# advimman/lama

Hardware: NVIDIA H100
Metric: images/sec FFCResNetGenerator @512x512 bs32 (higher is better)
Workload: dtype bf16x3(f32 accumulate)

## Files before the change

lama_b200/csrc/conv_tc.cu:

```cuda
#include <cuda.h>
#include <stdlib.h>

#include <type_traits>

#include "common.cuh"

namespace ffcb {
namespace {

constexpr int BM = 128;
constexpr int BK = 64;
constexpr int WG_K = 16;
constexpr int kThreads = 384;
constexpr int kConsumers = 256;
constexpr int kTileABytes = BM * BK * 2;
constexpr int kMaxStages = 8;
constexpr int kBarBytes = 1024;
constexpr int kSmemLimit = 227 * 1024;

struct TcParams {
  View out, addend;
  const float* shift;
  int N, act, addend_post;
  int BN, num_n_tiles;
  long long num_m_tiles;
  int stages;
  int flat;
  int TW, TH, tiles_x, tiles_y;
  int stride;
  int coord_off[2];
  int nseg;
  int a_il[2];
  const unsigned short* a_ptr[2];
  long long a_sg[2], a_lo[2];
  int a_tiles_per_image[2];
  int out_planar;
  int ring;
  int hints;
  int rr_dy0, rr_a_bytes, rr_w_bytes;
  int halo_a_bytes;
  signed char seg_taps[FFCB_MAX_KSEG];
  ffcb_kseg seg[FFCB_MAX_KSEG];
};

__device__ __forceinline__ uint32_t smem_u32(const void* p) { return (uint32_t)__cvta_generic_to_shared(p); }

__device__ __forceinline__ void mbar_init(uint64_t* bar, uint32_t count) {
  asm volatile("mbarrier.init.shared::cta.b64 [%0], %1;" ::"r"(smem_u32(bar)), "r"(count));
}
__device__ __forceinline__ void mbar_expect_tx(uint64_t* bar, uint32_t bytes) {
  asm volatile("mbarrier.arrive.expect_tx.shared::cta.b64 _, [%0], %1;" ::"r"(smem_u32(bar)), "r"(bytes) : "memory");
}
__device__ __forceinline__ void mbar_arrive(uint64_t* bar) {
  asm volatile("mbarrier.arrive.shared::cta.b64 _, [%0];" ::"r"(smem_u32(bar)) : "memory");
}
__device__ __forceinline__ void mbar_wait(uint64_t* bar, uint32_t parity) {
  asm volatile(
      "{\n\t"
      ".reg .pred p;\n\t"
      "WAIT_LOOP:\n\t"
      "mbarrier.try_wait.parity.shared::cta.b64 p, [%0], %1;\n\t"
      "@p bra WAIT_DONE;\n\t"
      "bra WAIT_LOOP;\n\t"
      "WAIT_DONE:\n\t"
      "}\n" ::"r"(smem_u32(bar)), "r"(parity)
      : "memory");
}

__device__ __forceinline__ void tma_load_3d(void* dst, const CUtensorMap* map, uint64_t* bar, int c0, int c1, int c2) {
  asm volatile(
      "cp.async.bulk.tensor.3d.shared::cluster.global.mbarrier::complete_tx::bytes [%0], [%1, {%3, %4, %5}], [%2];"
      ::"r"(smem_u32(dst)), "l"(map), "r"(smem_u32(bar)), "r"(c0), "r"(c1), "r"(c2)
      : "memory");
}
__device__ __forceinline__ void tma_load_5d(void* dst, const CUtensorMap* map, uint64_t* bar, int c0, int c1, int c2,
                                            int c3, int c4) {
  asm volatile(
      "cp.async.bulk.tensor.5d.shared::cluster.global.mbarrier::complete_tx::bytes [%0], [%1, {%3, %4, %5, %6, %7}], [%2];"
      ::"r"(smem_u32(dst)), "l"(map), "r"(smem_u32(bar)), "r"(c0), "r"(c1), "r"(c2), "r"(c3), "r"(c4)
      : "memory");
}

__device__ __forceinline__ void bulk_load(void* dst, const void* src, uint32_t bytes, uint64_t* bar) {
  asm volatile("cp.async.bulk.shared::cluster.global.mbarrier::complete_tx::bytes [%0], [%1], %2, [%3];"
               ::"r"(smem_u32(dst)), "l"(src), "r"(bytes), "r"(smem_u32(bar)) : "memory");
}

__device__ __forceinline__ void prefetch_tmap(const CUtensorMap* map) {
  asm volatile("prefetch.tensormap [%0];" ::"l"(map) : "memory");
}

constexpr uint32_t kLoSw = 1u << 16;
constexpr uint32_t kHiSw = (uint32_t)(1024 >> 4) | (1u << 30);
constexpr uint32_t kLoIl = (uint32_t)(2048 >> 4) << 16;
constexpr uint32_t kHiIl = (uint32_t)(128 >> 4);

__device__ __forceinline__ uint32_t desc_addr(uint32_t saddr) { return (saddr & 0x3FFFF) >> 4; }

__device__ __forceinline__ uint64_t desc64(uint32_t lo, uint32_t hi) {
  uint64_t d;
  asm("mov.b64 %0, {%1, %2};" : "=l"(d) : "r"(lo), "r"(hi));
  return d;
}
__device__ __forceinline__ bool elect_one() {
  uint32_t pred;
  asm volatile(
      "{\n\t"
      ".reg .pred P;\n\t"
      "elect.sync _|P, 0xffffffff;\n\t"
      "selp.b32 %0, 1, 0, P;\n\t"
      "}\n"
      : "=r"(pred));
  return pred != 0;
}

__device__ __forceinline__ void wgmma_fence() { asm volatile("wgmma.fence.sync.aligned;" ::: "memory"); }
__device__ __forceinline__ void wgmma_commit() { asm volatile("wgmma.commit_group.sync.aligned;" ::: "memory"); }
template <int N>
__device__ __forceinline__ void wgmma_wait() { asm volatile("wgmma.wait_group.sync.aligned %0;" ::"n"(N) : "memory"); }
template <int BN>
__device__ __forceinline__ void fence_acc(float* d) {
#pragma unroll
  for (int i = 0; i < BN / 2; ++i) asm volatile("" : "+f"(d[i])::"memory");
}

__device__ __forceinline__ void wgmma_n32(float* d, uint64_t da, uint64_t db, uint32_t scale_d) {
  asm volatile(
      "{\n\t.reg .pred p;\n\tsetp.ne.b32 p, %18, 0;\n\t"
      "wgmma.mma_async.sync.aligned.m64n32k16.f32.bf16.bf16 {"
      "%0, %1, %2, %3, %4, %5, %6, %7, %8, %9, %10, %11, %12, %13, %14, %15"
      "}, %16, %17, p, 1, 1, 0, 0;\n\t}\n"
      : "+f"(d[0]), "+f"(d[1]), "+f"(d[2]), "+f"(d[3]), "+f"(d[4]), "+f"(d[5]), "+f"(d[6]), "+f"(d[7]),
        "+f"(d[8]), "+f"(d[9]), "+f"(d[10]), "+f"(d[11]), "+f"(d[12]), "+f"(d[13]), "+f"(d[14]), "+f"(d[15])
      : "l"(da), "l"(db), "r"(scale_d));
}
__device__ __forceinline__ void wgmma_n64(float* d, uint64_t da, uint64_t db, uint32_t scale_d) {
  asm volatile(
      "{\n\t.reg .pred p;\n\tsetp.ne.b32 p, %34, 0;\n\t"
      "wgmma.mma_async.sync.aligned.m64n64k16.f32.bf16.bf16 {"
      "%0, %1, %2, %3, %4, %5, %6, %7, %8, %9, %10, %11, %12, %13, %14, %15, "
      "%16, %17, %18, %19, %20, %21, %22, %23, %24, %25, %26, %27, %28, %29, %30, %31"
      "}, %32, %33, p, 1, 1, 0, 0;\n\t}\n"
      : "+f"(d[0]), "+f"(d[1]), "+f"(d[2]), "+f"(d[3]), "+f"(d[4]), "+f"(d[5]), "+f"(d[6]), "+f"(d[7]),
        "+f"(d[8]), "+f"(d[9]), "+f"(d[10]), "+f"(d[11]), "+f"(d[12]), "+f"(d[13]), "+f"(d[14]), "+f"(d[15]),
        "+f"(d[16]), "+f"(d[17]), "+f"(d[18]), "+f"(d[19]), "+f"(d[20]), "+f"(d[21]), "+f"(d[22]), "+f"(d[23]),
        "+f"(d[24]), "+f"(d[25]), "+f"(d[26]), "+f"(d[27]), "+f"(d[28]), "+f"(d[29]), "+f"(d[30]), "+f"(d[31])
      : "l"(da), "l"(db), "r"(scale_d));
}
__device__ __forceinline__ void wgmma_n96(float* d, uint64_t da, uint64_t db, uint32_t scale_d) {
  asm volatile(
      "{\n\t.reg .pred p;\n\tsetp.ne.b32 p, %50, 0;\n\t"
      "wgmma.mma_async.sync.aligned.m64n96k16.f32.bf16.bf16 {"
      "%0, %1, %2, %3, %4, %5, %6, %7, %8, %9, %10, %11, %12, %13, %14, %15, "
      "%16, %17, %18, %19, %20, %21, %22, %23, %24, %25, %26, %27, %28, %29, %30, %31, "
      "%32, %33, %34, %35, %36, %37, %38, %39, %40, %41, %42, %43, %44, %45, %46, %47"
      "}, %48, %49, p, 1, 1, 0, 0;\n\t}\n"
      : "+f"(d[0]), "+f"(d[1]), "+f"(d[2]), "+f"(d[3]), "+f"(d[4]), "+f"(d[5]), "+f"(d[6]), "+f"(d[7]),
        "+f"(d[8]), "+f"(d[9]), "+f"(d[10]), "+f"(d[11]), "+f"(d[12]), "+f"(d[13]), "+f"(d[14]), "+f"(d[15]),
        "+f"(d[16]), "+f"(d[17]), "+f"(d[18]), "+f"(d[19]), "+f"(d[20]), "+f"(d[21]), "+f"(d[22]), "+f"(d[23]),
        "+f"(d[24]), "+f"(d[25]), "+f"(d[26]), "+f"(d[27]), "+f"(d[28]), "+f"(d[29]), "+f"(d[30]), "+f"(d[31]),
        "+f"(d[32]), "+f"(d[33]), "+f"(d[34]), "+f"(d[35]), "+f"(d[36]), "+f"(d[37]), "+f"(d[38]), "+f"(d[39]),
        "+f"(d[40]), "+f"(d[41]), "+f"(d[42]), "+f"(d[43]), "+f"(d[44]), "+f"(d[45]), "+f"(d[46]), "+f"(d[47])
      : "l"(da), "l"(db), "r"(scale_d));
}
__device__ __forceinline__ void wgmma_n128(float* d, uint64_t da, uint64_t db, uint32_t scale_d) {
  asm volatile(
      "{\n\t.reg .pred p;\n\tsetp.ne.b32 p, %66, 0;\n\t"
      "wgmma.mma_async.sync.aligned.m64n128k16.f32.bf16.bf16 {"
      "%0, %1, %2, %3, %4, %5, %6, %7, %8, %9, %10, %11, %12, %13, %14, %15, "
      "%16, %17, %18, %19, %20, %21, %22, %23, %24, %25, %26, %27, %28, %29, %30, %31, "
      "%32, %33, %34, %35, %36, %37, %38, %39, %40, %41, %42, %43, %44, %45, %46, %47, "
      "%48, %49, %50, %51, %52, %53, %54, %55, %56, %57, %58, %59, %60, %61, %62, %63"
      "}, %64, %65, p, 1, 1, 0, 0;\n\t}\n"
      : "+f"(d[0]), "+f"(d[1]), "+f"(d[2]), "+f"(d[3]), "+f"(d[4]), "+f"(d[5]), "+f"(d[6]), "+f"(d[7]),
        "+f"(d[8]), "+f"(d[9]), "+f"(d[10]), "+f"(d[11]), "+f"(d[12]), "+f"(d[13]), "+f"(d[14]), "+f"(d[15]),
        "+f"(d[16]), "+f"(d[17]), "+f"(d[18]), "+f"(d[19]), "+f"(d[20]), "+f"(d[21]), "+f"(d[22]), "+f"(d[23]),
        "+f"(d[24]), "+f"(d[25]), "+f"(d[26]), "+f"(d[27]), "+f"(d[28]), "+f"(d[29]), "+f"(d[30]), "+f"(d[31]),
        "+f"(d[32]), "+f"(d[33]), "+f"(d[34]), "+f"(d[35]), "+f"(d[36]), "+f"(d[37]), "+f"(d[38]), "+f"(d[39]),
        "+f"(d[40]), "+f"(d[41]), "+f"(d[42]), "+f"(d[43]), "+f"(d[44]), "+f"(d[45]), "+f"(d[46]), "+f"(d[47]),
        "+f"(d[48]), "+f"(d[49]), "+f"(d[50]), "+f"(d[51]), "+f"(d[52]), "+f"(d[53]), "+f"(d[54]), "+f"(d[55]),
        "+f"(d[56]), "+f"(d[57]), "+f"(d[58]), "+f"(d[59]), "+f"(d[60]), "+f"(d[61]), "+f"(d[62]), "+f"(d[63])
      : "l"(da), "l"(db), "r"(scale_d));
}
template <int BN>
__device__ __forceinline__ void wgmma_bn(float* d, uint64_t da, uint64_t db, uint32_t scale_d) {
  static_assert(BN == 32 || BN == 64 || BN == 96 || BN == 128, "N tile");
  if constexpr (BN == 32) wgmma_n32(d, da, db, scale_d);
  else if constexpr (BN == 64) wgmma_n64(d, da, db, scale_d);
  else if constexpr (BN == 96) wgmma_n96(d, da, db, scale_d);
  else wgmma_n128(d, da, db, scale_d);
}

struct TileCoord {
  int b, y0, x0;
  long long m0;
};

__device__ __forceinline__ TileCoord tile_coord(const TcParams& p, long long m_tile) {
  TileCoord t;
  if (p.flat) {
    t.m0 = m_tile * BM;
    t.b = 0; t.y0 = 0; t.x0 = 0;
  } else {
    const int per_img = p.tiles_x * p.tiles_y;
    t.b = (int)(m_tile / per_img);
    const int r = (int)(m_tile - (long long)t.b * per_img);
    t.y0 = (r / p.tiles_x) * p.TH;
    t.x0 = (r % p.tiles_x) * p.TW;
    t.m0 = 0;
  }
  return t;
}

template <bool IL, bool PO, bool RR, bool HALO, int BN>
__global__ void __launch_bounds__(kThreads, 1)
conv_tc_kernel(const __grid_constant__ TcParams p, const __grid_constant__ CUtensorMap map_in0,
               const __grid_constant__ CUtensorMap map_in1, const __grid_constant__ CUtensorMap map_w) {
  extern __shared__ __align__(1024) uint8_t smem_raw[];
  uint8_t* smem = reinterpret_cast<uint8_t*>((reinterpret_cast<uintptr_t>(smem_raw) + 1023) & ~(uintptr_t)1023);
  const int w_bytes = p.BN * BK * 2;
  const int stage_bytes = RR ? 2 * p.rr_a_bytes : HALO ? 2 * w_bytes : 2 * kTileABytes + 2 * w_bytes;
  uint8_t* w_res = smem;
  uint8_t* a_buf = smem;
  if constexpr (RR) smem += p.rr_w_bytes;
  if constexpr (HALO) smem += (size_t)4 * p.halo_a_bytes;
  uint64_t* bars = reinterpret_cast<uint64_t*>(smem + (size_t)p.stages * stage_bytes);
  uint64_t* full = bars;
  uint64_t* empty = bars + kMaxStages;
  uint64_t* w_bar = bars + 2 * kMaxStages;
  uint64_t* a_full = bars + 2 * kMaxStages + 1;
  uint64_t* a_empty = a_full + 2;

  const int warp = threadIdx.x >> 5, lane = threadIdx.x & 31;

  if (warp == 0 && lane == 0) {
    prefetch_tmap(&map_in0);
    prefetch_tmap(&map_in1);
    prefetch_tmap(&map_w);
  }
  if (warp == 1 && lane == 0) {
    for (int s = 0; s < p.stages; ++s) { mbar_init(&full[s], 1); mbar_init(&empty[s], kConsumers); }
    if constexpr (RR) mbar_init(w_bar, 1);
    if constexpr (HALO)
      for (int s = 0; s < 2; ++s) { mbar_init(&a_full[s], 1); mbar_init(&a_empty[s], kConsumers); }
    asm volatile("fence.mbarrier_init.release.cluster;" ::: "memory");
  }
  __syncthreads();

  int total_kblocks = 0;
  for (int s = 0; s < p.nseg; ++s) total_kblocks += (p.seg[s].nch + BK - 1) / BK;
  const long long num_tiles = p.num_m_tiles * p.num_n_tiles;

  if (warp == 0) {
    if constexpr (HALO) {
      int stage = 0, ast = 0;
      uint32_t phase = 0, aph = 0;
      for (long long t = blockIdx.x; t < num_tiles; t += gridDim.x) {
        const int n_tile = (int)(t % p.num_n_tiles);
        const TileCoord tc = tile_coord(p, t / p.num_n_tiles);
        int kofs = 0;
        for (int s = 0; s < p.nseg;) {
          const int ntap = p.seg_taps[s];
          const ffcb_kseg g = p.seg[s];
          const CUtensorMap* map = g.src ? &map_in1 : &map_in0;
          const int nblk = (g.nch + BK - 1) / BK;
          for (int j = 0; j < nblk; ++j) {
            for (int u = 0; u < (ntap == 9 ? 3 : 1); ++u) {
              const int dxu = ntap == 9 ? u - 1 : g.dx;
              mbar_wait(&a_empty[ast], aph ^ 1);
              if (elect_one()) {
                uint8_t* ab = a_buf + (size_t)ast * 2 * p.halo_a_bytes;
                mbar_expect_tx(&a_full[ast], 2u * p.TW * (p.TH + 2) * BK * 2);
                const int cx = tc.x0 + dxu + p.coord_off[g.src], cy = tc.y0 - 1 + p.coord_off[g.src];
                tma_load_5d(ab, map, &a_full[ast], g.c0 + j * BK, cx, cy, tc.b, 0);
                tma_load_5d(ab + p.halo_a_bytes, map, &a_full[ast], g.c0 + j * BK, cx, cy, tc.b, 1);
              }
              __syncwarp();
              if (++ast == 2) { ast = 0; aph ^= 1; }
              for (int tap = 0; tap < ntap; ++tap) {
                if (p.seg[s + tap].dx != dxu) continue;
                mbar_wait(&empty[stage], phase ^ 1);
                if (elect_one()) {
                  uint8_t* st = smem + (size_t)stage * stage_bytes;
                  mbar_expect_tx(&full[stage], (uint32_t)stage_bytes);
                  const int k = kofs + (tap * nblk + j) * BK;
                  tma_load_3d(st, &map_w, &full[stage], k, n_tile * p.BN, 0);
                  tma_load_3d(st + w_bytes, &map_w, &full[stage], k, n_tile * p.BN, 1);
                }
                __syncwarp();
                if (++stage == p.stages) { stage = 0; phase ^= 1; }
              }
            }
          }
          kofs += ntap * nblk * BK;
          s += ntap;
        }
      }
    } else if constexpr (RR) {
      const ffcb_kseg g0 = p.seg[0];
      const CUtensorMap* map = g0.src ? &map_in1 : &map_in0;
      if (elect_one()) {
        mbar_expect_tx(w_bar, (uint32_t)p.rr_w_bytes);
        for (int s = 0; s < p.nseg; ++s) {
          tma_load_3d(w_res + (size_t)s * 2 * w_bytes, &map_w, w_bar, s * BK, 0, 0);
          tma_load_3d(w_res + (size_t)s * 2 * w_bytes + w_bytes, &map_w, w_bar, s * BK, 0, 1);
        }
      }
      __syncwarp();
      int stage = 0;
      uint32_t phase = 0;
      for (long long t = blockIdx.x; t < num_tiles; t += gridDim.x) {
        const TileCoord tc = tile_coord(p, t);
        mbar_wait(&empty[stage], phase ^ 1);
        if (elect_one()) {
          uint8_t* st = smem + (size_t)stage * stage_bytes;
          mbar_expect_tx(&full[stage], (uint32_t)stage_bytes);
          const int cx = tc.x0 + g0.dx + p.coord_off[g0.src], cy = tc.y0 + p.rr_dy0 + p.coord_off[g0.src];
          tma_load_5d(st, map, &full[stage], g0.c0, cx, cy, tc.b, 0);
          tma_load_5d(st + p.rr_a_bytes, map, &full[stage], g0.c0, cx, cy, tc.b, 1);
        }
        __syncwarp();
        if (++stage == p.stages) { stage = 0; phase ^= 1; }
      }
    } else {
      int stage = 0;
      uint32_t phase = 0;
      for (long long t = blockIdx.x; t < num_tiles; t += gridDim.x) {
        const int n_tile = (int)(t % p.num_n_tiles);
        const TileCoord tc = tile_coord(p, t / p.num_n_tiles);
        int kb = 0;
        for (int s = 0; s < p.nseg; ++s) {
          const ffcb_kseg g = p.seg[s];
          const CUtensorMap* map = g.src ? &map_in1 : &map_in0;
          const int nblk = (g.nch + BK - 1) / BK;
          const int cx = tc.x0 * p.stride + g.dx + p.coord_off[g.src];
          const int cy = tc.y0 * p.stride + g.dy + p.coord_off[g.src];
          const int il = IL ? p.a_il[g.src] : 0;
          for (int j = 0; j < nblk; ++j, ++kb) {
            mbar_wait(&empty[stage], phase ^ 1);
            if (elect_one()) {
              uint8_t* st = smem + (size_t)stage * stage_bytes;
              mbar_expect_tx(&full[stage], (uint32_t)stage_bytes);
              const int cc = g.c0 + j * BK;
              if (IL && il) {
                const long long blk = p.flat ? (tc.m0 >> 7)
                                             : (long long)tc.b * p.a_tiles_per_image[g.src] + ((tc.y0 * p.out.W) >> 7);
                const unsigned short* src = p.a_ptr[g.src] + blk * p.a_sg[g.src] + (long long)(cc >> 3) * 1024;
                bulk_load(st, src, kTileABytes, &full[stage]);
                bulk_load(st + kTileABytes, src + p.a_lo[g.src], kTileABytes, &full[stage]);
              } else if (p.flat) {
                tma_load_3d(st, map, &full[stage], cc, (int)tc.m0, 0);
                tma_load_3d(st + kTileABytes, map, &full[stage], cc, (int)tc.m0, 1);
              } else {
                tma_load_5d(st, map, &full[stage], cc, cx, cy, tc.b, 0);
                tma_load_5d(st + kTileABytes, map, &full[stage], cc, cx, cy, tc.b, 1);
              }
              tma_load_3d(st + 2 * kTileABytes, &map_w, &full[stage], kb * BK, n_tile * p.BN, 0);
              tma_load_3d(st + 2 * kTileABytes + w_bytes, &map_w, &full[stage], kb * BK, n_tile * p.BN, 1);
            }
            __syncwarp();
            if (++stage == p.stages) { stage = 0; phase ^= 1; }
          }
        }
      }
    }
  } else if (warp >= 4) {
    const int g = (warp >> 2) - 1;
    const int w = warp & 3, q = lane & 3;
    const int row = g * 64 + w * 16 + (lane >> 2) + 8 * (q & 1);
    const int cb = 4 * (q >> 1);
    const bool odd = (q & 1) != 0;
    const uint32_t a_row_sw = (uint32_t)(g * 64 * BK * 2) >> 4;
    const uint32_t a_row_il = (uint32_t)(g * 64 * 16) >> 4;
    const int HW = p.out.H * p.out.W;
    const bool has_add = p.addend.ptr != nullptr;
    float acc[BN / 2];
#pragma unroll
    for (int i = 0; i < BN / 2; ++i) acc[i] = 0.f;
    int stage = 0, ast = 0;
    uint32_t phase = 0, aph = 0;
    const int a_row0 = (g + 1) * p.TW;
    if constexpr (RR) mbar_wait(w_bar, 0);
    for (long long t = blockIdx.x; t < num_tiles; t += gridDim.x) {
      const int n_tile = (int)(t % p.num_n_tiles);
      const TileCoord tc = tile_coord(p, t / p.num_n_tiles);
      fence_acc<BN>(acc);
      if constexpr (HALO) {
        int prev = -1, a_prev = -1, nt = 0;
        for (int s = 0; s < p.nseg;) {
          const int ntap = p.seg_taps[s];
          const int nblk = (p.seg[s].nch + BK - 1) / BK;
          for (int j = 0; j < nblk; ++j) {
            for (int u = 0; u < (ntap == 9 ? 3 : 1); ++u) {
              const int dxu = ntap == 9 ? u - 1 : p.seg[s].dx;
              mbar_wait(&a_full[ast], aph);
              const uint32_t ab = smem_u32(a_buf + (size_t)ast * 2 * p.halo_a_bytes);
              for (int tap = 0; tap < ntap; ++tap) {
                const int dy = p.seg[s + tap].dy;
                if (p.seg[s + tap].dx != dxu) continue;
                const uint32_t a_off = (uint32_t)((a_row0 + dy * p.TW) * (BK * 2)) >> 4;
                const uint32_t a_hi = desc_addr(ab) + a_off;
                const uint32_t a_lo = desc_addr(ab + (uint32_t)p.halo_a_bytes) + a_off;
                mbar_wait(&full[stage], phase);
                wgmma_fence();
                const uint32_t st = smem_u32(smem + (size_t)stage * stage_bytes);
                const uint32_t w_hi = desc_addr(st), w_lo = desc_addr(st + (uint32_t)w_bytes);
#pragma unroll
                for (int k = 0; k < BK / WG_K; ++k) {
                  const uint32_t adv = (uint32_t)((k * WG_K * 2) >> 4);
                  wgmma_bn<BN>(acc, desc64((a_hi + adv) | kLoSw, kHiSw), desc64((w_hi + adv) | kLoSw, kHiSw),
                               (nt | k) != 0);
                  wgmma_bn<BN>(acc, desc64((a_lo + adv) | kLoSw, kHiSw), desc64((w_hi + adv) | kLoSw, kHiSw), 1);
                  wgmma_bn<BN>(acc, desc64((a_hi + adv) | kLoSw, kHiSw), desc64((w_lo + adv) | kLoSw, kHiSw), 1);
                }
                wgmma_commit();
                wgmma_wait<1>();
                if (prev >= 0) mbar_arrive(&empty[prev]);
                prev = stage;
                if (++stage == p.stages) { stage = 0; phase ^= 1; }
                if (a_prev >= 0) { mbar_arrive(&a_empty[a_prev]); a_prev = -1; }
                ++nt;
              }
              a_prev = ast;
              if (++ast == 2) { ast = 0; aph ^= 1; }
            }
          }
          s += ntap;
        }
        wgmma_wait<0>();
        fence_acc<BN>(acc);
        mbar_arrive(&empty[prev]);
        mbar_arrive(&a_empty[a_prev]);
      } else if constexpr (RR) {
        mbar_wait(&full[stage], phase);
        const uint32_t st = smem_u32(smem + (size_t)stage * stage_bytes);
        const uint32_t wr = smem_u32(w_res);
        for (int sgi = 0; sgi < p.nseg; ++sgi) {
          wgmma_fence();
          const uint32_t a_off = (uint32_t)((p.seg[sgi].dy - p.rr_dy0) * p.TW * (BK * 2));
          const uint32_t a_hi = desc_addr(st + a_off) + a_row_sw;
          const uint32_t a_lo = desc_addr(st + a_off + (uint32_t)p.rr_a_bytes) + a_row_sw;
          const uint32_t w_hi = desc_addr(wr + (uint32_t)(sgi * 2 * w_bytes));
          const uint32_t w_lo = desc_addr(wr + (uint32_t)(sgi * 2 * w_bytes + w_bytes));
#pragma unroll
          for (int k = 0; k < BK / WG_K; ++k) {
            const uint32_t adv = (uint32_t)((k * WG_K * 2) >> 4);
            wgmma_bn<BN>(acc, desc64((a_hi + adv) | kLoSw, kHiSw), desc64((w_hi + adv) | kLoSw, kHiSw), (sgi | k) != 0);
            wgmma_bn<BN>(acc, desc64((a_lo + adv) | kLoSw, kHiSw), desc64((w_hi + adv) | kLoSw, kHiSw), 1);
            wgmma_bn<BN>(acc, desc64((a_hi + adv) | kLoSw, kHiSw), desc64((w_lo + adv) | kLoSw, kHiSw), 1);
          }
          wgmma_commit();
          wgmma_wait<1>();
        }
        wgmma_wait<0>();
        fence_acc<BN>(acc);
        mbar_arrive(&empty[stage]);
        if (++stage == p.stages) { stage = 0; phase ^= 1; }
      } else {
        int prev = -1, sgi = 0, j = 0;
        for (int kb = 0; kb < total_kblocks; ++kb) {
          const bool il = IL && p.a_il[p.seg[sgi].src] != 0;
          const uint32_t a_lodesc = il ? kLoIl : kLoSw, a_hidesc = il ? kHiIl : kHiSw;
          const uint32_t a_row = il ? a_row_il : a_row_sw;
          const uint32_t a_step = il ? (uint32_t)(4096 >> 4) : (uint32_t)((WG_K * 2) >> 4);
          if (IL && ++j == (p.seg[sgi].nch + BK - 1) / BK) { ++sgi; j = 0; }
          mbar_wait(&full[stage], phase);
          wgmma_fence();
          const uint32_t st = smem_u32(smem + (size_t)stage * stage_bytes);
          const uint32_t a_hi = desc_addr(st) + a_row;
          const uint32_t a_lo = desc_addr(st + kTileABytes) + a_row;
          const uint32_t w_hi = desc_addr(st + 2 * kTileABytes);
          const uint32_t w_lo = desc_addr(st + 2 * kTileABytes + w_bytes);
#pragma unroll
          for (int k = 0; k < BK / WG_K; ++k) {
            const uint32_t wadv = (uint32_t)((k * WG_K * 2) >> 4);
            const uint32_t aadv = (uint32_t)k * a_step;
            wgmma_bn<BN>(acc, desc64((a_hi + aadv) | a_lodesc, a_hidesc), desc64((w_hi + wadv) | kLoSw, kHiSw),
                         (kb | k) != 0);
            wgmma_bn<BN>(acc, desc64((a_lo + aadv) | a_lodesc, a_hidesc), desc64((w_hi + wadv) | kLoSw, kHiSw), 1);
            wgmma_bn<BN>(acc, desc64((a_hi + aadv) | a_lodesc, a_hidesc), desc64((w_lo + wadv) | kLoSw, kHiSw), 1);
          }
          wgmma_commit();
          wgmma_wait<1>();
          if (prev >= 0) mbar_arrive(&empty[prev]);
          prev = stage;
          if (++stage == p.stages) { stage = 0; phase ^= 1; }
        }
        wgmma_wait<0>();
        fence_acc<BN>(acc);
        mbar_arrive(&empty[prev]);
      }

      int b, y, x;
      bool valid;
      if (p.flat) {
        const unsigned m = (unsigned)tc.m0 + (unsigned)row;
        valid = m < (unsigned)(p.out.B * HW);
        const unsigned mm = valid ? m : 0u;
        b = (int)(mm / (unsigned)HW);
        const unsigned r = mm - (unsigned)b * (unsigned)HW;
        y = (int)(r / (unsigned)p.out.W);
        x = (int)(r - (unsigned)y * (unsigned)p.out.W);
      } else {
        b = tc.b;
        y = tc.y0 + row / p.TW;
        x = tc.x0 + row % p.TW;
        valid = y < p.out.H && x < p.out.W;
      }
      const long long o_out = valid ? pix_off(p.out, b, y, x) : 0;
      const long long o_add = (has_add && valid) ? pix_off(p.addend, b, y, x) : 0;
      int mir_dy = 0, mir_dx = 0;
      if (!PO && p.ring && valid) {
        int my, mx;
        if (ring_mirrors(p.out, y, x, my, mx)) {
          if (my != -2) mir_dy = (my - y) * (int)p.out.sy;
          if (mx != -2) mir_dx = (mx - x) * (int)p.out.sx;
        }
      }
      const uint64_t pol = l2_policy(PO && p.hints ? 2 : 0);
#pragma unroll
      for (int j = 0; j < BN / 8; ++j) {
        const float s0 = odd ? acc[4 * j] : acc[4 * j + 2], s1 = odd ? acc[4 * j + 1] : acc[4 * j + 3];
        const float r0 = __shfl_xor_sync(0xffffffffu, s0, 1), r1 = __shfl_xor_sync(0xffffffffu, s1, 1);
        float4 v = odd ? make_float4(r0, r1, acc[4 * j + 2], acc[4 * j + 3])
                       : make_float4(acc[4 * j], acc[4 * j + 1], r0, r1);
        const int n = n_tile * p.BN + 8 * j + cb;
        if (!valid || n >= p.N) continue;
        if (p.shift != nullptr) {
          const float4 sh = __ldg(reinterpret_cast<const float4*>(p.shift + n));
          v.x += sh.x; v.y += sh.y; v.z += sh.z; v.w += sh.w;
        }
        float4 ad = make_float4(0.f, 0.f, 0.f, 0.f);
        if (has_add) ad = load4(p.addend, o_add + n);
        if (!p.addend_post) { v.x += ad.x; v.y += ad.y; v.z += ad.z; v.w += ad.w; }
        if (p.act == FFCB_ACT_RELU) {
          v.x = fmaxf(v.x, 0.f); v.y = fmaxf(v.y, 0.f); v.z = fmaxf(v.z, 0.f); v.w = fmaxf(v.w, 0.f);
        } else if (p.act != FFCB_ACT_NONE) {
          v.x = slow_act(v.x, p.act); v.y = slow_act(v.y, p.act); v.z = slow_act(v.z, p.act); v.w = slow_act(v.w, p.act);
        }
        if (p.addend_post) { v.x += ad.x; v.y += ad.y; v.z += ad.z; v.w += ad.w; }
        if constexpr (PO) {
          st_hint_f4(reinterpret_cast<float*>(p.out.ptr) + o_out + chan_off(p.out, n), v, pol);
        } else {
          store4(p.out, o_out + n, v);
          if (mir_dy) store4(p.out, o_out + mir_dy + n, v);
          if (mir_dx) store4(p.out, o_out + mir_dx + n, v);
          if (mir_dy && mir_dx) store4(p.out, o_out + mir_dy + mir_dx + n, v);
        }
      }
    }
  }
}

typedef CUresult (*EncodeTiledFn)(CUtensorMap*, CUtensorMapDataType, cuuint32_t, void*, const cuuint64_t*,
                                  const cuuint64_t*, const cuuint32_t*, const cuuint32_t*, CUtensorMapInterleave,
                                  CUtensorMapSwizzle, CUtensorMapL2promotion, CUtensorMapFloatOOBfill);

EncodeTiledFn get_encode() {
  static EncodeTiledFn fn = nullptr;
  if (fn == nullptr) {
    void* p = nullptr;
    cudaDriverEntryPointQueryResult q;
    if (cudaGetDriverEntryPoint("cuTensorMapEncodeTiled", &p, cudaEnableDefault, &q) == cudaSuccess &&
        q == cudaDriverEntryPointSuccess)
      fn = reinterpret_cast<EncodeTiledFn>(p);
  }
  return fn;
}

int encode_typed(CUtensorMap* map, void* base, CUtensorMapDataType dt, CUtensorMapSwizzle sw, int rank,
                 const cuuint64_t* dims, const cuuint64_t* strides_bytes, const cuuint32_t* box, const cuuint32_t* estr,
                 const char* what) {
  EncodeTiledFn fn = get_encode();
  if (fn == nullptr) {
    set_error("conv(tc): cuTensorMapEncodeTiled entry point unavailable");
    return FFCB_ECUDA;
  }
  CUresult r = fn(map, dt, (cuuint32_t)rank, base, dims, strides_bytes, box, estr, CU_TENSOR_MAP_INTERLEAVE_NONE, sw,
                  CU_TENSOR_MAP_L2_PROMOTION_L2_256B, CU_TENSOR_MAP_FLOAT_OOB_FILL_NONE);
  if (r != CUDA_SUCCESS) {
    set_error("conv(tc): cuTensorMapEncodeTiled(%s) failed with CUresult %d (rank %d, dims %llu %llu %llu, box %u %u %u)",
              what, (int)r, rank, (unsigned long long)dims[0], (unsigned long long)dims[1],
              (unsigned long long)(rank > 2 ? dims[2] : 0), box[0], box[1], rank > 2 ? box[2] : 0);
    return FFCB_ECUDA;
  }
  return FFCB_OK;
}

int encode(CUtensorMap* map, void* base, int rank, const cuuint64_t* dims, const cuuint64_t* strides_bytes,
           const cuuint32_t* box, const cuuint32_t* estr, const char* what) {
  return encode_typed(map, base, CU_TENSOR_MAP_DATA_TYPE_BFLOAT16, CU_TENSOR_MAP_SWIZZLE_128B, rank, dims, strides_bytes,
                      box, estr, what);
}

int pick_bn(int n) {
  if (const char* e = getenv("FFCB_TC_BN")) {
    const int v = atoi(e);
    if (v >= 32 && v <= 128 && v % 32 == 0) return v < n ? v : (n + 31) / 32 * 32;
  }
  if (n <= 128) return (n + 31) / 32 * 32;
  if (n == 192) return 96;
  return 128;
}

}

int conv_tc(const ffcb_conv_desc* d, cudaStream_t stream) {
  FFCB_REQUIRE(d->out.B > 0, "conv(tc): empty batch");
  FFCB_REQUIRE((long long)d->out.B * d->out.H * d->out.W < (1ll << 31), "conv(tc): more than 2^31 output pixels");
  bool used[2] = {false, false}, taps[2] = {false, false};
  int reach[2] = {0, 0};
  for (int i = 0; i < d->nseg; ++i) {
    used[d->seg[i].src] = true;
    if (d->seg[i].dx != 0 || d->seg[i].dy != 0) taps[d->seg[i].src] = true;
    const int ax = d->seg[i].dx < 0 ? -d->seg[i].dx : d->seg[i].dx, ay = d->seg[i].dy < 0 ? -d->seg[i].dy : d->seg[i].dy;
    if (ax > reach[d->seg[i].src]) reach[d->seg[i].src] = ax;
    if (ay > reach[d->seg[i].src]) reach[d->seg[i].src] = ay;
    FFCB_REQUIRE(d->seg[i].c0 % 8 == 0, "conv(tc): segment %d starts at channel %d (must be a multiple of 8)", i,
                 d->seg[i].c0);
  }
  for (int s = 0; s < 2; ++s) {
    if (!used[s]) continue;
    const ffcb_tensor& t = d->in[s];
    FFCB_REQUIRE(t.fmt == FFCB_BF16X2, "conv(tc): in[%d] must be split bf16 (FFCB_BF16X2)", s);
    if (t.cg != 0) {
      FFCB_REQUIRE(t.cg == 8 && t.tile == 128 && !taps[s] && d->stride == 1 && t.H == d->out.H && t.W == d->out.W,
                   "conv(tc): a channel-group planar in[%d] must be tile-blocked (tile=128, cg=8) with 1x1 taps, stride 1",
                   s);
      for (int i = 0; i < d->nseg; ++i)
        if (d->seg[i].src == s)
// ... 112 lines not shown
    p.num_m_tiles = (long long)d->out.B * p.tiles_x * p.tiles_y;
    p.halo_a_bytes = p.TW * (p.TH + 2) * BK * 2;
  } else {
    int tw = 1;
    while (tw < W && tw < BM) tw <<= 1;
    p.TW = tw; p.TH = BM / tw;
    p.tiles_x = (W + p.TW - 1) / p.TW;
    p.tiles_y = (H + p.TH - 1) / p.TH;
    p.num_m_tiles = (long long)d->out.B * p.tiles_x * p.tiles_y;
    FFCB_REQUIRE(p.TW * d->stride <= 256 && p.TH * d->stride <= 256, "conv(tc): tile exceeds the TMA box limit");
  }

  for (int s = 0; s < 2; ++s)
    if (p.a_il[s] && !flat)
      FFCB_REQUIRE(p.TW == W && p.TW * p.TH == BM && H % p.TH == 0 && (H * W) % BM == 0,
                   "conv(tc): tile-blocked in[%d] in a spatial contraction needs M tiles of whole rows (W a power of two "
                   "<= 128 dividing 128, H*W a multiple of 128); got %dx%d", s, H, W);

  alignas(64) CUtensorMap maps[3];
  int rc;
  for (int s = 0; s < 2; ++s) {
    if (!used[s]) { p.coord_off[s] = 0; continue; }
    const ffcb_tensor& t = d->in[s];
    const cuuint64_t esz = 2;
    if (p.a_il[s]) { p.coord_off[s] = 0; continue; }
    if (flat) {
      cuuint64_t dims[3] = {(cuuint64_t)t.C, (cuuint64_t)t.B * t.H * t.W, 2};
      cuuint64_t str[2] = {(cuuint64_t)t.sx * esz, (cuuint64_t)t.lo_off * esz};
      cuuint32_t box[3] = {BK, BM, 1}, es[3] = {1, 1, 1};
      p.coord_off[s] = 0;
      if ((rc = encode(&maps[s], t.ptr, 3, dims, str, box, es, "flat activations"))) return rc;
    } else {
      const bool ring = taps[s] && d->border == FFCB_BORDER_REFLECT;
      const int off = ring ? t.pad : 0;
      char* base = (char*)t.ptr - (int64_t)off * ((int64_t)t.sy + t.sx) * (int64_t)esz;
      cuuint64_t dims[5] = {(cuuint64_t)t.C, (cuuint64_t)(t.W + 2 * off), (cuuint64_t)(t.H + 2 * off),
                            (cuuint64_t)t.B, 2};
      cuuint64_t str[4] = {(cuuint64_t)t.sx * esz, (cuuint64_t)t.sy * esz, (cuuint64_t)t.sb * esz,
                           (cuuint64_t)t.lo_off * esz};
      cuuint32_t box[5] = {BK, (cuuint32_t)(p.TW * d->stride), (cuuint32_t)(p.TH * d->stride), 1, 1};
      if (rr) box[2] = (cuuint32_t)(p.TH + rr_dy_max - rr_dy_min);
      if (halo) box[2] = (cuuint32_t)(p.TH + 2);
      cuuint32_t es[5] = {1, (cuuint32_t)d->stride, (cuuint32_t)d->stride, 1, 1};
      p.coord_off[s] = off;
      if ((rc = encode(&maps[s], base, 5, dims, str, box, es, "spatial activations"))) return rc;
    }
  }
  {
    cuuint64_t dims[3] = {(cuuint64_t)kpad, (cuuint64_t)d->n_out, 2};
    cuuint64_t str[2] = {(cuuint64_t)kpad * 2, (cuuint64_t)kpad * d->n_out * 2};
    cuuint32_t box[3] = {BK, (cuuint32_t)p.BN, 1}, es[3] = {1, 1, 1};
    FFCB_REQUIRE(((uintptr_t)d->weight % 16) == 0, "conv(tc): weight pointer not 16-byte aligned");
    if ((rc = encode(&maps[2], const_cast<void*>(d->weight), 3, dims, str, box, es, "weights"))) return rc;
  }

  for (int s = 0; s < 2; ++s)
    if (!used[s] || p.a_il[s]) maps[s] = maps[2];
  if (d->out.cg == 0) {
    const ffcb_tensor& t = d->out;
    const cuuint64_t esz = t.fmt == FFCB_BF16X2 ? 2 : 4;
    FFCB_REQUIRE(((uintptr_t)t.ptr % 16) == 0 && (t.sx * esz) % 16 == 0 && (t.sy * esz) % 16 == 0 &&
                     (t.sb * esz) % 16 == 0 && (esz == 4 || (t.lo_off * esz) % 16 == 0),
                 "conv(tc): out strides / pointer not 16-byte aligned (C must be a multiple of %d)", esz == 2 ? 8 : 4);
  }

  const int stage_bytes = rr ? 2 * p.rr_a_bytes : halo ? 2 * p.BN * BK * 2 : 2 * kTileABytes + 2 * p.BN * BK * 2;
  const int bar_bytes = kBarBytes + (rr ? p.rr_w_bytes : 0) + (halo ? 4 * p.halo_a_bytes : 0);
  int stages = (kSmemLimit - 1024 - bar_bytes) / stage_bytes;
  if (stages > kMaxStages) stages = kMaxStages;
  FFCB_REQUIRE(stages >= 2, "conv(tc): BN=%d leaves fewer than 2 pipeline stages", p.BN);
  p.stages = stages;
  const size_t smem = (size_t)stages * stage_bytes + bar_bytes + 1024;
  int dev = 0, sms = 132;
  FFCB_CUDA(cudaGetDevice(&dev));
  FFCB_CUDA(cudaDeviceGetAttribute(&sms, cudaDevAttrMultiProcessorCount, dev));
  const long long tiles = p.num_m_tiles * p.num_n_tiles;
  const int grid = (int)(tiles < sms ? tiles : sms);
  const bool any_il = p.a_il[0] || p.a_il[1];
  auto launch = [&](auto kernel) -> int {
    FFCB_CUDA(cudaFuncSetAttribute(kernel, cudaFuncAttributeMaxDynamicSharedMemorySize, kSmemLimit));
    kernel<<<grid, kThreads, smem, stream>>>(p, maps[0], maps[1], maps[2]);
    return FFCB_OK;
  };
  auto launch_bn = [&](auto bn) -> int {
    constexpr int N = decltype(bn)::value;
    if (rr) return launch(conv_tc_kernel<false, false, true, false, N>);
    if (halo) return launch(conv_tc_kernel<false, false, false, true, N>);
    if (any_il)
      return p.out_planar ? launch(conv_tc_kernel<true, true, false, false, N>)
                          : launch(conv_tc_kernel<true, false, false, false, N>);
    return p.out_planar ? launch(conv_tc_kernel<false, true, false, false, N>)
                        : launch(conv_tc_kernel<false, false, false, false, N>);
  };
  switch (p.BN) {
    case 32: rc = launch_bn(std::integral_constant<int, 32>()); break;
    case 64: rc = launch_bn(std::integral_constant<int, 64>()); break;
    case 96: rc = launch_bn(std::integral_constant<int, 96>()); break;
    default: rc = launch_bn(std::integral_constant<int, 128>()); break;
  }
  if (rc) return rc;
  FFCB_LAUNCH_CHECK("conv_tc_kernel");
  return FFCB_OK;
}

}
```

Baseline: 314.7.

## Add ping-pong consumer warpgroup schedule with register reallocation to tensor-core conv

For flat and row-reuse conv modes, the two consumer warpgroups now each own whole 128-row tiles and alternate tiles, rather than splitting one tile's rows. Named barriers order their MMA phases so one warpgroup's epilogue overlaps the other's mainloop. Producer warps drop registers via setmaxnreg and consumers raise theirs to hold two accumulator sets. The goal is to hide epilogue cost behind tensor-core work, at the price of doubled accumulator registers and more complex ring/phase bookkeeping.

Result: no change. 316.0, median of 6 (+0.4%).

```diff
diff --git a/lama_b200/csrc/conv_tc.cu b/lama_b200/csrc/conv_tc.cu
--- a/lama_b200/csrc/conv_tc.cu
+++ b/lama_b200/csrc/conv_tc.cu
@@ -4,6 +4,7 @@
 #include <type_traits>
 
 #include "common.cuh"
+#include "conv_tc_sched.cuh"
 
 namespace ffcb {
 namespace {
@@ -12,7 +13,9 @@
 constexpr int BK = 64;
 constexpr int WG_K = 16;
 constexpr int kThreads = 384;
-constexpr int kConsumers = 256;
+constexpr int kProducerRegs = 40;
+constexpr int kConsumerRegs = 232;
+constexpr int kOrderBar = 1;
 constexpr int kTileABytes = BM * BK * 2;
 constexpr int kMaxStages = 8;
 constexpr int kBarBytes = 1024;
@@ -114,6 +117,13 @@
   return pred != 0;
 }
 
+template <int N>
+__device__ __forceinline__ void setmaxnreg_dec() { asm volatile("setmaxnreg.dec.sync.aligned.u32 %0;" ::"n"(N)); }
+template <int N>
+__device__ __forceinline__ void setmaxnreg_inc() { asm volatile("setmaxnreg.inc.sync.aligned.u32 %0;" ::"n"(N)); }
+__device__ __forceinline__ void order_bar_sync(int id) { asm volatile("bar.sync %0, 256;" ::"r"(id) : "memory"); }
+__device__ __forceinline__ void order_bar_arrive(int id) { asm volatile("bar.arrive %0, 256;" ::"r"(id) : "memory"); }
+
 __device__ __forceinline__ void wgmma_fence() { asm volatile("wgmma.fence.sync.aligned;" ::: "memory"); }
 __device__ __forceinline__ void wgmma_commit() { asm volatile("wgmma.commit_group.sync.aligned;" ::: "memory"); }
 template <int N>
@@ -212,7 +222,7 @@
   return t;
 }
 
-template <bool IL, bool PO, bool RR, bool HALO, int BN>
+template <bool IL, bool PO, bool RR, bool HALO, bool PP, int BN>
 __global__ void __launch_bounds__(kThreads, 1)
 conv_tc_kernel(const __grid_constant__ TcParams p, const __grid_constant__ CUtensorMap map_in0,
                const __grid_constant__ CUtensorMap map_in1, const __grid_constant__ CUtensorMap map_w) {
@@ -239,19 +249,21 @@
     prefetch_tmap(&map_w);
   }
   if (warp == 1 && lane == 0) {
-    for (int s = 0; s < p.stages; ++s) { mbar_init(&full[s], 1); mbar_init(&empty[s], kConsumers); }
+    const uint32_t releasers = PP ? tcs::kWgThreads : 2 * tcs::kWgThreads;
+    for (int s = 0; s < p.stages; ++s) { mbar_init(&full[s], 1); mbar_init(&empty[s], releasers); }
     if constexpr (RR) mbar_init(w_bar, 1);
     if constexpr (HALO)
-      for (int s = 0; s < 2; ++s) { mbar_init(&a_full[s], 1); mbar_init(&a_empty[s], kConsumers); }
+      for (int s = 0; s < 2; ++s) { mbar_init(&a_full[s], 1); mbar_init(&a_empty[s], releasers); }
     asm volatile("fence.mbarrier_init.release.cluster;" ::: "memory");
   }
   __syncthreads();
 
-  int total_kblocks = 0;
-  for (int s = 0; s < p.nseg; ++s) total_kblocks += (p.seg[s].nch + BK - 1) / BK;
+  static_assert(!(PP && HALO), "the column-halo mode runs the cooperative schedule only");
   const long long num_tiles = p.num_m_tiles * p.num_n_tiles;
 
-  if (warp == 0) {
+  if (warp < 4) {
+    if constexpr (PP) setmaxnreg_dec<kProducerRegs>();
+    if (warp != 0) return;
     if constexpr (HALO) {
       int stage = 0, ast = 0;
       uint32_t phase = 0, aph = 0;
@@ -364,27 +376,37 @@
         }
       }
     }
-  } else if (warp >= 4) {
+  } else {
+    if constexpr (PP) setmaxnreg_inc<kConsumerRegs>();
     const int g = (warp >> 2) - 1;
+    constexpr int RB = PP ? 2 : 1;
     const int w = warp & 3, q = lane & 3;
-    const int row = g * 64 + w * 16 + (lane >> 2) + 8 * (q & 1);
+    const int row0 = w * 16 + (lane >> 2) + 8 * (q & 1);
     const int cb = 4 * (q >> 1);
     const bool odd = (q & 1) != 0;
-    const uint32_t a_row_sw = (uint32_t)(g * 64 * BK * 2) >> 4;
-    const uint32_t a_row_il = (uint32_t)(g * 64 * 16) >> 4;
     const int HW = p.out.H * p.out.W;
     const bool has_add = p.addend.ptr != nullptr;
-    float acc[BN / 2];
-#pragma unroll
-    for (int i = 0; i < BN / 2; ++i) acc[i] = 0.f;
-    int stage = 0, ast = 0;
-    uint32_t phase = 0, aph = 0;
+    float acc[RB][BN / 2];
+#pragma unroll
+    for (int rb = 0; rb < RB; ++rb)
+#pragma unroll
+      for (int i = 0; i < BN / 2; ++i) acc[rb][i] = 0.f;
+    const int kblocks = tcs::kblocks_per_tile(p.seg, p.nseg, BK);
+    const int per_tile = RR ? 1 : kblocks;
+    tcs::Ring sr = PP ? tcs::wg_ring_start(g, p.stages, per_tile) : tcs::Ring{0, 0u};
+    int ast = 0;
+    uint32_t aph = 0;
     const int a_row0 = (g + 1) * p.TW;
     if constexpr (RR) mbar_wait(w_bar, 0);
-    for (long long t = blockIdx.x; t < num_tiles; t += gridDim.x) {
+    const long long t_first = PP ? tcs::wg_first_tile(blockIdx.x, gridDim.x, g) : (long long)blockIdx.x;
+    const long long t_step = PP ? tcs::wg_tile_step(gridDim.x) : (long long)gridDim.x;
+    for (long long t = t_first; t < num_tiles; t += t_step) {
       const int n_tile = (int)(t % p.num_n_tiles);
       const TileCoord tc = tile_coord(p, t / p.num_n_tiles);
-      fence_acc<BN>(acc);
+#pragma unroll
+      for (int rb = 0; rb < RB; ++rb) fence_acc<BN>(acc[rb]);
+      if (PP && tcs::order_wait(t, blockIdx.x)) order_bar_sync(kOrderBar + g);
+      const bool signal = PP && tcs::order_signal(t, gridDim.x, num_tiles);
       if constexpr (HALO) {
         int prev = -1, a_prev = -1, nt = 0;
         for (int s = 0; s < p.nseg;) {
@@ -401,23 +423,23 @@
                 const uint32_t a_off = (uint32_t)((a_row0 + dy * p.TW) * (BK * 2)) >> 4;
                 const uint32_t a_hi = desc_addr(ab) + a_off;
                 const uint32_t a_lo = desc_addr(ab + (uint32_t)p.halo_a_bytes) + a_off;
-                mbar_wait(&full[stage], phase);
+                mbar_wait(&full[sr.slot], sr.phase);
                 wgmma_fence();
-                const uint32_t st = smem_u32(smem + (size_t)stage * stage_bytes);
+                const uint32_t st = smem_u32(smem + (size_t)sr.slot * stage_bytes);
                 const uint32_t w_hi = desc_addr(st), w_lo = desc_addr(st + (uint32_t)w_bytes);
 #pragma unroll
                 for (int k = 0; k < BK / WG_K; ++k) {
                   const uint32_t adv = (uint32_t)((k * WG_K * 2) >> 4);
-                  wgmma_bn<BN>(acc, desc64((a_hi + adv) | kLoSw, kHiSw), desc64((w_hi + adv) | kLoSw, kHiSw),
+                  wgmma_bn<BN>(acc[0], desc64((a_hi + adv) | kLoSw, kHiSw), desc64((w_hi + adv) | kLoSw, kHiSw),
                                (nt | k) != 0);
-                  wgmma_bn<BN>(acc, desc64((a_lo + adv) | kLoSw, kHiSw), desc64((w_hi + adv) | kLoSw, kHiSw), 1);
-                  wgmma_bn<BN>(acc, desc64((a_hi + adv) | kLoSw, kHiSw), desc64((w_lo + adv) | kLoSw, kHiSw), 1);
+                  wgmma_bn<BN>(acc[0], desc64((a_lo + adv) | kLoSw, kHiSw), desc64((w_hi + adv) | kLoSw, kHiSw), 1);
+                  wgmma_bn<BN>(acc[0], desc64((a_hi + adv) | kLoSw, kHiSw), desc64((w_lo + adv) | kLoSw, kHiSw), 1);
                 }
                 wgmma_commit();
                 wgmma_wait<1>();
                 if (prev >= 0) mbar_arrive(&empty[prev]);
-                prev = stage;
-                if (++stage == p.stages) { stage = 0; phase ^= 1; }
+                prev = sr.slot;
+                tcs::ring_step(sr, p.stages);
                 if (a_prev >= 0) { mbar_arrive(&a_empty[a_prev]); a_prev = -1; }
                 ++nt;
               }
@@ -428,124 +450,144 @@
           s += ntap;
         }
         wgmma_wait<0>();
-        fence_acc<BN>(acc);
+        fence_acc<BN>(acc[0]);
         mbar_arrive(&empty[prev]);
         mbar_arrive(&a_empty[a_prev]);
       } else if constexpr (RR) {
-        mbar_wait(&full[stage], phase);
-        const uint32_t st = smem_u32(smem + (size_t)stage * stage_bytes);
+        mbar_wait(&full[sr.slot], sr.phase);
+        const uint32_t st = smem_u32(smem + (size_t)sr.slot * stage_bytes);
         const uint32_t wr = smem_u32(w_res);
         for (int sgi = 0; sgi < p.nseg; ++sgi) {
           wgmma_fence();
           const uint32_t a_off = (uint32_t)((p.seg[sgi].dy - p.rr_dy0) * p.TW * (BK * 2));
-          const uint32_t a_hi = desc_addr(st + a_off) + a_row_sw;
-          const uint32_t a_lo = desc_addr(st + a_off + (uint32_t)p.rr_a_bytes) + a_row_sw;
+          const uint32_t a_hi = desc_addr(st + a_off);
+          const uint32_t a_lo = desc_addr(st + a_off + (uint32_t)p.rr_a_bytes);
           const uint32_t w_hi = desc_addr(wr + (uint32_t)(sgi * 2 * w_bytes));
           const uint32_t w_lo = desc_addr(wr + (uint32_t)(sgi * 2 * w_bytes + w_bytes));
 #pragma unroll
           for (int k = 0; k < BK / WG_K; ++k) {
             const uint32_t adv = (uint32_t)((k * WG_K * 2) >> 4);
-            wgmma_bn<BN>(acc, desc64((a_hi + adv) | kLoSw, kHiSw), desc64((w_hi + adv) | kLoSw, kHiSw), (sgi | k) != 0);
-            wgmma_bn<BN>(acc, desc64((a_lo + adv) | kLoSw, kHiSw), desc64((w_hi + adv) | kLoSw, kHiSw), 1);
-            wgmma_bn<BN>(acc, desc64((a_hi + adv) | kLoSw, kHiSw), desc64((w_lo + adv) | kLoSw, kHiSw), 1);
+#pragma unroll
+            for (int rb = 0; rb < RB; ++rb) {
+              const uint32_t aadv = adv + ((uint32_t)((PP ? rb : g) * 64 * BK * 2) >> 4);
+              wgmma_bn<BN>(acc[rb], desc64((a_hi + aadv) | kLoSw, kHiSw), desc64((w_hi + adv) | kLoSw, kHiSw),
+                           (sgi | k) != 0);
+              wgmma_bn<BN>(acc[rb], desc64((a_lo + aadv) | kLoSw, kHiSw), desc64((w_hi + adv) | kLoSw, kHiSw), 1);
+              wgmma_bn<BN>(acc[rb], desc64((a_hi + aadv) | kLoSw, kHiSw), desc64((w_lo + adv) | kLoSw, kHiSw), 1);
+            }
           }
           wgmma_commit();
           wgmma_wait<1>();
         }
+        if (signal) order_bar_arrive(kOrderBar + (g ^ 1));
         wgmma_wait<0>();
-        fence_acc<BN>(acc);
-        mbar_arrive(&empty[stage]);
-        if (++stage == p.stages) { stage = 0; phase ^= 1; }
+#pragma unroll
+        for (int rb = 0; rb < RB; ++rb) fence_acc<BN>(acc[rb]);
+        mbar_arrive(&empty[sr.slot]);
+        tcs::ring_step(sr, p.stages);
       } else {
         int prev = -1, sgi = 0, j = 0;
-        for (int kb = 0; kb < total_kblocks; ++kb) {
+        for (int kb = 0; kb < kblocks; ++kb) {
           const bool il = IL && p.a_il[p.seg[sgi].src] != 0;
           const uint32_t a_lodesc = il ? kLoIl : kLoSw, a_hidesc = il ? kHiIl : kHiSw;
-          const uint32_t a_row = il ? a_row_il : a_row_sw;
+          const uint32_t a_rb = il ? (uint32_t)(64 * 16) >> 4 : (uint32_t)(64 * BK * 2) >> 4;
           const uint32_t a_step = il ? (uint32_t)(4096 >> 4) : (uint32_t)((WG_K * 2) >> 4);
           if (IL && ++j == (p.seg[sgi].nch + BK - 1) / BK) { ++sgi; j = 0; }
-          mbar_wait(&full[stage], phase);
+          mbar_wait(&full[sr.slot], sr.phase);
           wgmma_fence();
-          const uint32_t st = smem_u32(smem + (size_t)stage * stage_bytes);
-          const uint32_t a_hi = desc_addr(st) + a_row;
-          const uint32_t a_lo = desc_addr(st + kTileABytes) + a_row;
+          const uint32_t st = smem_u32(smem + (size_t)sr.slot * stage_bytes);
+          const uint32_t a_hi = desc_addr(st);
+          const uint32_t a_lo = desc_addr(st + kTileABytes);
           const uint32_t w_hi = desc_addr(st + 2 * kTileABytes);
           const uint32_t w_lo = desc_addr(st + 2 * kTileABytes + w_bytes);
 #pragma unroll
           for (int k = 0; k < BK / WG_K; ++k) {
             const uint32_t wadv = (uint32_t)((k * WG_K * 2) >> 4);
-            const uint32_t aadv = (uint32_t)k * a_step;
-            wgmma_bn<BN>(acc, desc64((a_hi + aadv) | a_lodesc, a_hidesc), desc64((w_hi + wadv) | kLoSw, kHiSw),
-                         (kb | k) != 0);
-            wgmma_bn<BN>(acc, desc64((a_lo + aadv) | a_lodesc, a_hidesc), desc64((w_hi + wadv) | kLoSw, kHiSw), 1);
-            wgmma_bn<BN>(acc, desc64((a_hi + aadv) | a_lodesc, a_hidesc), desc64((w_lo + wadv) | kLoSw, kHiSw), 1);
+#pragma unroll
+            for (int rb = 0; rb < RB; ++rb) {
+              const uint32_t aadv = (uint32_t)k * a_step + (uint32_t)(PP ? rb : g) * a_rb;
+              wgmma_bn<BN>(acc[rb], desc64((a_hi + aadv) | a_lodesc, a_hidesc), desc64((w_hi + wadv) | kLoSw, kHiSw),
+                           (kb | k) != 0);
+              wgmma_bn<BN>(acc[rb], desc64((a_lo + aadv) | a_lodesc, a_hidesc), desc64((w_hi + wadv) | kLoSw, kHiSw),
+                           1);
+              wgmma_bn<BN>(acc[rb], desc64((a_hi + aadv) | a_lodesc, a_hidesc), desc64((w_lo + wadv) | kLoSw, kHiSw),
+                           1);
+            }
           }
           wgmma_commit();
           wgmma_wait<1>();
           if (prev >= 0) mbar_arrive(&empty[prev]);
-          prev = stage;
-          if (++stage == p.stages) { stage = 0; phase ^= 1; }
-        }
+          prev = sr.slot;
+          tcs::ring_step(sr, p.stages);
+        }
+        if (signal) order_bar_arrive(kOrderBar + (g ^ 1));
         wgmma_wait<0>();
-        fence_acc<BN>(acc);
+#pragma unroll
+        for (int rb = 0; rb < RB; ++rb) fence_acc<BN>(acc[rb]);
         mbar_arrive(&empty[prev]);
       }
-
-      int b, y, x;
-      bool valid;
-      if (p.flat) {
-        const unsigned m = (unsigned)tc.m0 + (unsigned)row;
-        valid = m < (unsigned)(p.out.B * HW);
-        const unsigned mm = valid ? m : 0u;
-        b = (int)(mm / (unsigned)HW);
-        const unsigned r = mm - (unsigned)b * (unsigned)HW;
-        y = (int)(r / (unsigned)p.out.W);
-        x = (int)(r - (unsigned)y * (unsigned)p.out.W);
-      } else {
-        b = tc.b;
-        y = tc.y0 + row / p.TW;
-        x = tc.x0 + row % p.TW;
-        valid = y < p.out.H && x < p.out.W;
-      }
-      const long long o_out = valid ? pix_off(p.out, b, y, x) : 0;
-      const long long o_add = (has_add && valid) ? pix_off(p.addend, b, y, x) : 0;
-      int mir_dy = 0, mir_dx = 0;
-      if (!PO && p.ring && valid) {
-        int my, mx;
-        if (ring_mirrors(p.out, y, x, my, mx)) {
-          if (my != -2) mir_dy = (my - y) * (int)p.out.sy;
-          if (mx != -2) mir_dx = (mx - x) * (int)p.out.sx;
-        }
-      }
-      const uint64_t pol = l2_policy(PO && p.hints ? 2 : 0);
-#pragma unroll
-      for (int j = 0; j < BN / 8; ++j) {
-        const float s0 = odd ? acc[4 * j] : acc[4 * j + 2], s1 = odd ? acc[4 * j + 1] : acc[4 * j + 3];
-        const float r0 = __shfl_xor_sync(0xffffffffu, s0, 1), r1 = __shfl_xor_sync(0xffffffffu, s1, 1);
-        float4 v = odd ? make_float4(r0, r1, acc[4 * j + 2], acc[4 * j + 3])
-                       : make_float4(acc[4 * j], acc[4 * j + 1], r0, r1);
-        const int n = n_tile * p.BN + 8 * j + cb;
-        if (!valid || n >= p.N) continue;
-        if (p.shift != nullptr) {
-          const float4 sh = __ldg(reinterpret_cast<const float4*>(p.shift + n));
-          v.x += sh.x; v.y += sh.y; v.z += sh.z; v.w += sh.w;
-        }
-        float4 ad = make_float4(0.f, 0.f, 0.f, 0.f);
-        if (has_add) ad = load4(p.addend, o_add + n);
-        if (!p.addend_post) { v.x += ad.x; v.y += ad.y; v.z += ad.z; v.w += ad.w; }
-        if (p.act == FFCB_ACT_RELU) {
-          v.x = fmaxf(v.x, 0.f); v.y = fmaxf(v.y, 0.f); v.z = fmaxf(v.z, 0.f); v.w = fmaxf(v.w, 0.f);
-        } else if (p.act != FFCB_ACT_NONE) {
-          v.x = slow_act(v.x, p.act); v.y = slow_act(v.y, p.act); v.z = slow_act(v.z, p.act); v.w = slow_act(v.w, p.act);
-        }
-        if (p.addend_post) { v.x += ad.x; v.y += ad.y; v.z += ad.z; v.w += ad.w; }
-        if constexpr (PO) {
-          st_hint_f4(reinterpret_cast<float*>(p.out.ptr) + o_out + chan_off(p.out, n), v, pol);
+      if constexpr (PP) tcs::ring_skip(sr, p.stages, per_tile);
+
+#pragma unroll
+      for (int rb = 0; rb < RB; ++rb) {
+        const int row = (PP ? rb : g) * 64 + row0;
+        int b, y, x;
+        bool valid;
+        if (p.flat) {
+          const unsigned m = (unsigned)tc.m0 + (unsigned)row;
+          valid = m < (unsigned)(p.out.B * HW);
+          const unsigned mm = valid ? m : 0u;
+          b = (int)(mm / (unsigned)HW);
+          const unsigned r = mm - (unsigned)b * (unsigned)HW;
+          y = (int)(r / (unsigned)p.out.W);
+          x = (int)(r - (unsigned)y * (unsigned)p.out.W);
         } else {
-          store4(p.out, o_out + n, v);
-          if (mir_dy) store4(p.out, o_out + mir_dy + n, v);
-          if (mir_dx) store4(p.out, o_out + mir_dx + n, v);
-          if (mir_dy && mir_dx) store4(p.out, o_out + mir_dy + mir_dx + n, v);
+          b = tc.b;
+          y = tc.y0 + row / p.TW;
+          x = tc.x0 + row % p.TW;
+          valid = y < p.out.H && x < p.out.W;
+        }
+        const long long o_out = valid ? pix_off(p.out, b, y, x) : 0;
+        const long long o_add = (has_add && valid) ? pix_off(p.addend, b, y, x) : 0;
+        int mir_dy = 0, mir_dx = 0;
+        if (!PO && p.ring && valid) {
+          int my, mx;
+          if (ring_mirrors(p.out, y, x, my, mx)) {
+            if (my != -2) mir_dy = (my - y) * (int)p.out.sy;
+            if (mx != -2) mir_dx = (mx - x) * (int)p.out.sx;
+          }
+        }
+        const uint64_t pol = l2_policy(PO && p.hints ? 2 : 0);
+        const float* a = acc[rb];
+#pragma unroll
+        for (int j = 0; j < BN / 8; ++j) {
+          const float s0 = odd ? a[4 * j] : a[4 * j + 2], s1 = odd ? a[4 * j + 1] : a[4 * j + 3];
+          const float r0 = __shfl_xor_sync(0xffffffffu, s0, 1), r1 = __shfl_xor_sync(0xffffffffu, s1, 1);
+          float4 v = odd ? make_float4(r0, r1, a[4 * j + 2], a[4 * j + 3]) : make_float4(a[4 * j], a[4 * j + 1], r0, r1);
+          const int n = n_tile * p.BN + 8 * j + cb;
+          if (!valid || n >= p.N) continue;
+          if (p.shift != nullptr) {
+            const float4 sh = __ldg(reinterpret_cast<const float4*>(p.shift + n));
+            v.x += sh.x; v.y += sh.y; v.z += sh.z; v.w += sh.w;
+          }
+          float4 ad = make_float4(0.f, 0.f, 0.f, 0.f);
+          if (has_add) ad = load4(p.addend, o_add + n);
+          if (!p.addend_post) { v.x += ad.x; v.y += ad.y; v.z += ad.z; v.w += ad.w; }
+          if (p.act == FFCB_ACT_RELU) {
+            v.x = fmaxf(v.x, 0.f); v.y = fmaxf(v.y, 0.f); v.z = fmaxf(v.z, 0.f); v.w = fmaxf(v.w, 0.f);
+          } else if (p.act != FFCB_ACT_NONE) {
+            v.x = slow_act(v.x, p.act); v.y = slow_act(v.y, p.act); v.z = slow_act(v.z, p.act);
+            v.w = slow_act(v.w, p.act);
+          }
+          if (p.addend_post) { v.x += ad.x; v.y += ad.y; v.z += ad.z; v.w += ad.w; }
+          if constexpr (PO) {
+            st_hint_f4(reinterpret_cast<float*>(p.out.ptr) + o_out + chan_off(p.out, n), v, pol);
+          } else {
+            store4(p.out, o_out + n, v);
+            if (mir_dy) store4(p.out, o_out + mir_dy + n, v);
+            if (mir_dx) store4(p.out, o_out + mir_dx + n, v);
+            if (mir_dy && mir_dx) store4(p.out, o_out + mir_dy + mir_dx + n, v);
+          }
         }
       }
     }
@@ -824,15 +866,23 @@
     kernel<<<grid, kThreads, smem, stream>>>(p, maps[0], maps[1], maps[2]);
     return FFCB_OK;
   };
+  const bool pp = flat || rr;
   auto launch_bn = [&](auto bn) -> int {
     constexpr int N = decltype(bn)::value;
-    if (rr) return launch(conv_tc_kernel<false, false, true, false, N>);
-    if (halo) return launch(conv_tc_kernel<false, false, false, true, N>);
+    if (rr) return launch(conv_tc_kernel<false, false, true, false, true, N>);
+    if (halo) return launch(conv_tc_kernel<false, false, false, true, false, N>);
+    if (pp) {
+      if (any_il)
+        return p.out_planar ? launch(conv_tc_kernel<true, true, false, false, true, N>)
+                            : launch(conv_tc_kernel<true, false, false, false, true, N>);
+      return p.out_planar ? launch(conv_tc_kernel<false, true, false, false, true, N>)
+                          : launch(conv_tc_kernel<false, false, false, false, true, N>);
+    }
     if (any_il)
-      return p.out_planar ? launch(conv_tc_kernel<true, true, false, false, N>)
-                          : launch(conv_tc_kernel<true, false, false, false, N>);
-    return p.out_planar ? launch(conv_tc_kernel<false, true, false, false, N>)
-                        : launch(conv_tc_kernel<false, false, false, false, N>);
+      return p.out_planar ? launch(conv_tc_kernel<true, true, false, false, false, N>)
+                          : launch(conv_tc_kernel<true, false, false, false, false, N>);
+    return p.out_planar ? launch(conv_tc_kernel<false, true, false, false, false, N>)
+                        : launch(conv_tc_kernel<false, false, false, false, false, N>);
   };
   switch (p.BN) {
     case 32: rc = launch_bn(std::integral_constant<int, 32>()); break;
diff --git a/lama_b200/csrc/conv_tc_sched.cuh b/lama_b200/csrc/conv_tc_sched.cuh
--- /dev/null
+++ b/lama_b200/csrc/conv_tc_sched.cuh
@@ -0,0 +1,48 @@
+#pragma once
+#include <stdint.h>
+
+#if defined(__CUDACC__)
+#define FFCB_HD __host__ __device__ __forceinline__
+#else
+#define FFCB_HD inline
+#endif
+
+namespace ffcb {
+namespace tcs {
+
+constexpr int kWgThreads = 128;
+
+struct Ring {
+  int slot;
+  uint32_t phase;
+};
+
+FFCB_HD void ring_step(Ring& r, int n) {
+  if (++r.slot == n) { r.slot = 0; r.phase ^= 1u; }
+}
+FFCB_HD void ring_skip(Ring& r, int n, int by) {
+  const int s = r.slot + by, q = s / n;
+  r.slot = s - q * n;
+  r.phase ^= (uint32_t)q & 1u;
+}
+
+FFCB_HD long long wg_first_tile(int cta, int grid, int g) { return cta + (long long)g * grid; }
+FFCB_HD long long wg_tile_step(int grid) { return 2ll * grid; }
+FFCB_HD Ring wg_ring_start(int g, int n, int per_tile) {
+  Ring r{0, 0u};
+  ring_skip(r, n, g * per_tile);
+  return r;
+}
+
+FFCB_HD bool order_wait(long long t, int cta) { return t != cta; }
+FFCB_HD bool order_signal(long long t, int grid, long long num_tiles) { return t + grid < num_tiles; }
+
+template <class Seg>
+FFCB_HD int kblocks_per_tile(const Seg* seg, int nseg, int bk) {
+  int n = 0;
+  for (int s = 0; s < nseg; ++s) n += (seg[s].nch + bk - 1) / bk;
+  return n;
+}
+
+}
+}
```
